# Zhang-Xiaoxue/Senquential-Convex-Programming-for-Trajectory-Planning

Measured on AMD Instinct MI355X. Metric: SCP-QP solves/sec/GPU (4 veh, Hp=20); traj ℓ∞ err vs CVXOPT, higher is better.
Workload: dtype f64; 1 GPU; c2: 4-vehicle circle/crossing, Hp=20, batch=1024 noise seeds per GPU, full SCP solve per problem; n_veh=4, hp=20, batch_per_gpu=1024, parallelism=1 independent shards (no collective)

## Files before the change

### senquential-convex-programming-for-trajectory-planning_amd/csrc/scpqp_kernel.h

```cpp

#pragma once

#include <hip/hip_runtime.h>

#include <math.h>
#include <stdint.h>
#include <stdio.h>
#include <stdlib.h>
#include <string.h>

#include <new>
#include <type_traits>
#include <utility>

#include "scpqp.h"

#define NT 256
#define TXD 16
#define TYD (NT / TXD)
#define NWAVE (NT / 64)
#define SCR_PER_WAVE 640

namespace {

// ... 675 lines not shown
            if (lane < 2 && act) L.p0[(v * Hb + k) * 2 + lane] = cur;
        }
        bar();
    }
    for (int e = tid; e < V * Hb; e += NT) {
        const int v = e / Hb, l = e % Hb;
        double acc = 0.0;
        for (int k = l; k < Hb; ++k) {
            const double qk = (k == Hb - 1) ? P.Qf[v] : P.Q[v];
            const ldouble* gg = L.g + (v * Hb + k - l) * 2;
            const double ex = L.ref[(v * Hb + k) * 2] - L.p0[(v * Hb + k) * 2];
            const double ey = L.ref[(v * Hb + k) * 2 + 1] - L.p0[(v * Hb + k) * 2 + 1];
            acc += qk * (gg[0] * ex + gg[1] * ey);
        }
        L.qs[e] = P.uLim * (-2.0 * acc);
    }
    for (int r = tid; r < L.m; r += NT) {
        int i, j, o, k;
        if (r < L.mp) {
            const int pi = r / Hb;
            k = r % Hb;
            int ii = 0, rem = pi;
            while (rem >= V - 1 - ii) { rem -= V - 1 - ii; ++ii; }
            i = ii;
            j = ii + 1 + rem;
            o = -1;
        } else {
            const int ro = r - L.mp;
            const int vo = ro / Hb;
            k = ro % Hb;
            i = vo / O;
            o = vo % O;
            j = -1;
        }
        L.rinfo[r] = i | ((j + 1) << 8) | ((o + 1) << 16) | (k << 24);
    }
    bar();
    return sflag;
}

template <bool HG, bool VG, int RM, int OCC, int SH>
__device__ __noinline__ int setup_problem_ni(const cKArgs* ap, const cParams* Pp, gdouble* ws, int b, int Hb) {
    ap = (const cKArgs*)readfirstlane_u64((unsigned long long)ap);
    Pp = (const cParams*)readfirstlane_u64((unsigned long long)Pp);
    ws = (gdouble*)readfirstlane_u64((unsigned long long)ws);
    b = __builtin_amdgcn_readfirstlane(b);
    Hb = __builtin_amdgcn_readfirstlane(Hb);
    const cKArgs& a = *ap;
    const cParams& P = *Pp;
    const Off f = plan_offsets(shapeV<SH>(P.nV), shapeO<SH>(P.nO), shapeHM<SH>(P.hpMax), HG, VG, lean_plan(HG, VG, OCC));
    const Lay<HG, VG, RM, OCC> L = make_lay<HG, VG, RM, OCC, SH>(lds_base(), ws, f, P.nV, P.nO, Hb);
    return setup_problem(a, P, L, b);
}

constexpr int kSplit = 3, kPerWave = 21, kPerPass = kPerWave * NWAVE;
template <class TermSum, class Fn>
__device__ __forceinline__ void split3_outputs(int nout, TermSum part, Fn fn, int w) {
    const int lane = threadIdx.x & 63;
    const int j = lane / kSplit, sidx = lane - j * kSplit;
    for (int base = 0; base < nout; base += kPerPass) {
        const int e = base + w * kPerWave + j;
        const bool valid = lane < kSplit * kPerWave && e < nout;
        double2v acc = valid ? part(e, sidx) : double2v{0.0, 0.0};
        const double x1 = __shfl_down(acc.x, 1), y1 = __shfl_down(acc.y, 1);
        const double x2 = __shfl_down(acc.x, 2), y2 = __shfl_down(acc.y, 2);
        if (valid && sidx == 0) fn(e, double2v{acc.x + x1 + x2, acc.y + y1 + y2});
    }
}
template <class TermSum, class Fn>
__device__ __forceinline__ void split3_outputs(int nout, TermSum part, Fn fn) {
    split3_outputs(nout, part, fn, (int)(threadIdx.x >> 6));
}

template <class LT, class PX, class PY>
__device__ __forceinline__ void toeplitz_apply(const LT& L, PX x, PY y) {
    split3_outputs(
        L.V * L.Hb,
        [&](int e, int sidx) {
            const int v = e / L.Hb, k = e - v * L.Hb;
            const ldouble* gv = L.g + v * L.Hb * 2;
            const int xb = v * L.Hb;
            double a0 = 0.0, a1 = 0.0;
            for (int l = sidx; l <= k; l += kSplit) {
                const double xl = x[xb + l];
                const double2v gl = ld2(gv + (k - l) * 2);
                a0 += gl.x * xl;
                a1 += gl.y * xl;
            }
            return double2v{a0, a1};
        },
        [&](int e, double2v r) { st2(y + 2 * e, r); });
}

template <class LT, class PY, class Fn>
__device__ __forceinline__ void toeplitz_t_apply(const LT& L, PY y, Fn out, int w) {
    split3_outputs(
        L.V * L.Hb,
        [&](int e, int sidx) {
            const int v = e / L.Hb, l = e - v * L.Hb;
            const ldouble* gv = L.g + v * L.Hb * 2;
            const int yb = v * L.Hb * 2;
            double acc = 0.0;
            for (int k = l + sidx; k < L.Hb; k += kSplit)
                acc += gv[(k - l) * 2] * y[yb + 2 * k] + gv[(k - l) * 2 + 1] * y[yb + 2 * k + 1];
            return double2v{acc, 0.0};
        },
        [&](int e, double2v r) { out(e, r.x); }, w);
}
template <class LT, class PY, class Fn>
__device__ __forceinline__ void toeplitz_t_apply(const LT& L, PY y, Fn out) {
    toeplitz_t_apply(L, y, out, (int)(threadIdx.x >> 6));
}

template <class LT, class F>
__device__ __forceinline__ void incident_sum(const LT& L, int v, int k, F coef, double& s0,
                                            double& s1) {
    s0 = 0.0;
    s1 = 0.0;
    for (int w = 0; w < L.V; ++w) {
        if (w == v) continue;
        const int i = v < w ? v : w, j = v < w ? w : v;
        const int r = pair_index(i, j, L.V) * L.Hb + k;
        const double c = (v == i ? -1.0 : 1.0) * coef(r);
        s0 += c * L.rowE[2 * r];
        s1 += c * L.rowE[2 * r + 1];
    }
    for (int o = 0; o < L.O; ++o) {
        const int r = L.mp + (v * L.O + o) * L.Hb + k;
        const double c = -coef(r);
        s0 += c * L.rowE[2 * r];
        s1 += c * L.rowE[2 * r + 1];
    }
}

template <class LT, class PX>
__device__ __forceinline__ double gx_row(const LT& L, PX xu, double xw, int r) {
    if (r < L.m) {
        int i, j, o, k;
        row_decode(L.rinfo[r], i, j, o, k);
        const double e0 = L.rowE[2 * r], e1 = L.rowE[2 * r + 1];
        double val = -(e0 * L.ya[(i * L.Hb + k) * 2] + e1 * L.ya[(i * L.Hb + k) * 2 + 1]);
        if (j >= 0) val += e0 * L.ya[(j * L.Hb + k) * 2] + e1 * L.ya[(j * L.Hb + k) * 2 + 1];
        return val + L.rowW[r] * xw;
    }
    if (r < L.m + L.N) return xu[r - L.m];
    if (r < L.m + 2 * L.N) return -xu[r - L.m - L.N];
    return -xw;
}

template <class LT, class PT>
__device__ __forceinline__ double gt_incident_part(const LT& L, PT t, int vt) {
    double wsum = 0.0;
    for (int e = vt; e < L.V * L.Hb; e += NT) {
        const int v = e / L.Hb, k = e % L.Hb;
        double s0, s1;
        incident_sum(L, v, k, [&](int r) { return t[r]; }, s0, s1);
        L.yb[2 * e] = s0;
        L.yb[2 * e + 1] = s1;
    }
    for (int r = vt; r < L.m; r += NT) wsum += t[r] * L.rowW[r];
    return wsum;
}
template <class LT, class PT, class Fin>
__device__ __forceinline__ void gt_toeplitz_part(const LT& L, PT t, Fin fin, int vw) {
    toeplitz_t_apply(L, L.yb, [&](int e, double tt) { fin(e, tt + t[L.m + e] - t[L.m + L.N + e]); }, vw);
}
template <int BUF, class LT, class PT, class Fin>
__device__ double gt_apply_fin(const LT& L, PT t, Fin fin) {
    const int tid = threadIdx.x;
    const double wsum = gt_incident_part(L, t, tid);
    double red[4] = {wsum, 0.0, 0.0, 0.0};
    block_reduce4<1, BUF>(red, 0, L.red);
    gt_toeplitz_part(L, t, fin, tid >> 6);
    return red[0] - t[L.mc - 1];
}

template <class LT, class PT, class Fin, class FinW>
struct GtSide {
    static constexpr int STAGES = 2;
    const LT& L;
    PT t;
    Fin fin;
    FinW finw;
    __device__ __forceinline__ void operator()(int stage, int h, int nh) const {
        const int lane = threadIdx.x & 63;
        ldouble* part = L.red + kSidePart;
        for (int vw = h; vw < NWAVE; vw += nh) {
            if (stage == 0) {
                const double ws = wave_sum(gt_incident_part(L, t, vw * 64 + lane));
                if (lane == 0) part[vw] = ws;
            } else {
                gt_toeplitz_part(L, t, fin, vw);
                if (vw == 0 && lane == 0) {
                    double r = part[0];
#pragma unroll
                    for (int ww = 1; ww < NWAVE; ++ww) r = r + part[ww];
                    finw(r - t[L.mc - 1]);
                }
            }
        }
    }
};
template <class LT, class PT, class Fin, class FinW>
__device__ __forceinline__ GtSide<LT, PT, Fin, FinW> gt_side(const LT& L, PT t, Fin fin, FinW finw) {
    return GtSide<LT, PT, Fin, FinW>{L, t, fin, finw};
}

template <int TS, class LT, class PD>
__device__ __forceinline__ void assemble_tiles(const cParams& P, const LT& L, PD d, double rho) {
    const int tid = threadIdx.x, V = L.V, Hb = L.Hb, nb = L.nb, N = L.N;
    const double u2 = P.uLim * P.uLim;
    const int TH = (Hb + TS - 1) / TS, TD = TH * (TH + 1) / 2, TO = TH * TH;
    const int PV = V * (V - 1) / 2;
    const int ntile = V * TD + PV * TO;
    const double2v zero2 = {0.0, 0.0};
    for (int r0 = 0; r0 < ntile; r0 += NT) {
        const int t = r0 + (((r0 / NT) & 1) ? NT - 1 - tid : tid);
        if (t >= ntile) continue;
        int a_, b_, lt, mt;
        tile_decode(t, V, PV, a_, b_, lt, mt);
        const int l0 = TS * lt, m0 = TS * mt, k0 = l0 > m0 ? l0 : m0;
        const ldouble* ga = L.g + a_ * Hb * 2;
        const ldouble* gb = L.g + b_ * Hb * 2;
        const auto* W = L.Wt + 4 * (a_ * (a_ + 1) / 2 + b_);
        double2v av[TS], bv[TS];
#pragma unroll
        for (int i = 0; i < TS; ++i) {
            const int ia = k0 - 1 - l0 - i, ib = k0 - 1 - m0 - i;
            av[i] = ia >= 0 ? ld2(ga + 2 * ia) : zero2;
            bv[i] = ib >= 0 ? ld2(gb + 2 * ib) : zero2;
        }
        double c[TS][TS];
#pragma unroll
        for (int i = 0; i < TS; ++i)
#pragma unroll
            for (int j = 0; j < TS; ++j) c[i][j] = 0.0;
        double2v an = ld2(ga + 2 * (k0 - l0)), bn = ld2(gb + 2 * (k0 - m0));
        double2v wn0 = ld2(W + 4 * k0 * nb), wn1 = ld2(W + 4 * k0 * nb + 2);
        constexpr bool PF2 = LT::HGLOBAL;
        double2v an2 = an, bn2 = bn, wm0 = wn0, wm1 = wn1;
        if constexpr (PF2) {
            const int k1 = k0 + 1 < Hb ? k0 + 1 : k0;
            an2 = ld2(ga + 2 * (k1 - l0));
            bn2 = ld2(gb + 2 * (k1 - m0));
            wm0 = ld2(W + 4 * k1 * nb);
            wm1 = ld2(W + 4 * k1 * nb + 2);
        }
        auto trip = [&](const double2v& anew, const double2v& bnew, const double2v& w0,
                        const double2v& w1) {
#pragma unroll
            for (int i = TS - 1; i > 0; --i) {
                av[i] = av[i - 1];
                bv[i] = bv[i - 1];
            }
            av[0] = anew;
            bv[0] = bnew;
            double px[TS], py[TS];
#pragma unroll
            for (int j = 0; j < TS; ++j) {
                px[j] = w0.x * bv[j].x + w0.y * bv[j].y;
                py[j] = w1.x * bv[j].x + w1.y * bv[j].y;
            }
#pragma unroll
            for (int i = 0; i < TS; ++i)
#pragma unroll
                for (int j = 0; j < TS; ++j) c[i][j] = fma(av[i].y, py[j], fma(av[i].x, px[j], c[i][j]));
        };
#pragma unroll 2
        for (int k = k0; k < Hb; ++k) {
            const double2v acur = an, bcur = bn, w0 = wn0, w1 = wn1;
            if constexpr (PF2) {
                an = an2;
                bn = bn2;
                wn0 = wm0;
                wn1 = wm1;
                const int kn = k + 2 < Hb ? k + 2 : Hb - 1;
                an2 = ld2(ga + 2 * (kn - l0));
                bn2 = ld2(gb + 2 * (kn - m0));
                wm0 = ld2(W + 4 * kn * nb);
                wm1 = ld2(W + 4 * kn * nb + 2);
            } else {
                const int kn = k + 1 < Hb ? k + 1 : k;
                an = ld2(ga + 2 * (kn - l0));
                bn = ld2(gb + 2 * (kn - m0));
                wn0 = ld2(W + 4 * kn * nb);
                wn1 = ld2(W + 4 * kn * nb + 2);
            }
            trip(acur, bcur, w0, w1);
        }
#pragma unroll
        for (int di = 0; di < TS; ++di)
#pragma unroll
            for (int dj = 0; dj < TS; ++dj) {
                const int l = l0 + di, lp = m0 + dj;
                if (l >= Hb || lp >= Hb || (a_ == b_ && lp > l)) continue;
                const int row = a_ * Hb + l, col = b_ * Hb + lp;
                double acc = c[di][dj];
                if (row == col) acc += 2.0 * u2 * P.R[a_] + d[L.m + row] + d[L.m + N + row] + rho;
                L.H[roff(row) + col] = acc;
            }
    }
}

template <class LT, class PD>
__device__ void assemble(const cParams& P, const LT& L, PD d, double rho) {
    const int tid = threadIdx.x, V = L.V, Hb = L.Hb, nb = L.nb;
    const double u2 = P.uLim * P.uLim;
    const int nW = Hb * nb;
    PROF_T0_FINE();
    for (int e = tid; e < nW + V * Hb; e += NT) {
        if (e < nW) {
            const int k = e / nb, ab = e % nb;
            int a_ = 0;
            while ((a_ + 1) * (a_ + 2) / 2 <= ab) ++a_;
            const int b_ = ab - a_ * (a_ + 1) / 2;
            double w00 = 0.0, w01 = 0.0, w11 = 0.0;
            if (a_ == b_) {
                const double qk = 2.0 * u2 * ((k == Hb - 1) ? P.Qf[a_] : P.Q[a_]);
                w00 = qk;
                w11 = qk;
                for (int wv = 0; wv < V; ++wv) {
                    if (wv == a_) continue;
                    const int i = a_ < wv ? a_ : wv, j = a_ < wv ? wv : a_;
                    const int r = pair_index(i, j, V) * Hb + k;
                    const double e0 = L.rowE[2 * r], e1 = L.rowE[2 * r + 1], dr = d[r];
                    w00 += dr * e0 * e0;
                    w01 += dr * e0 * e1;
                    w11 += dr * e1 * e1;
                }
                for (int o = 0; o < L.O; ++o) {
                    const int r = L.mp + (a_ * L.O + o) * Hb + k;
                    const double e0 = L.rowE[2 * r], e1 = L.rowE[2 * r + 1], dr = d[r];
                    w00 += dr * e0 * e0;
                    w01 += dr * e0 * e1;
                    w11 += dr * e1 * e1;
                }
            } else {
                const int r = pair_index(b_, a_, V) * Hb + k;
                const double e0 = L.rowE[2 * r], e1 = L.rowE[2 * r + 1], dr = -d[r];
                w00 = dr * e0 * e0;
                w01 = dr * e0 * e1;
                w11 = dr * e1 * e1;
            }
            auto* W = L.Wt + 4 * e;
            W[0] = w00; W[1] = w01; W[2] = w01; W[3] = w11;
        } else {
            const int q = e - nW, v = q / Hb, k = q % Hb;
            double s0, s1;
            incident_sum(L, v, k, [&](int r) { return d[r] * L.rowW[r]; }, s0, s1);
            L.yb[2 * q] = s0;
            L.yb[2 * q + 1] = s1;
        }
    }
    double ww = 0.0;
    for (int r = tid; r < L.m; r += NT) ww += d[r] * L.rowW[r] * L.rowW[r];
    double red[4] = {ww, 0.0, 0.0, 0.0};
    block_reduce4<1, 2>(red, 0, L.red);
    PROF_ACC_FINE0(25);
    const int T4 = (Hb + 3) >> 2, PV = V * (V - 1) / 2;
    if constexpr (LT::HGLOBAL) {
        if (V * (T4 * (T4 + 1) / 2) + PV * T4 * T4 >= 2 * NT) assemble_tiles<4>(P, L, d, rho);
        else assemble_tiles<2>(P, L, d, rho);
    } else {
        (void)T4;
        (void)PV;
        assemble_tiles<4>(P, L, d, rho);
#ifdef SCPQP_DIAG_X2_ASM
        assemble_tiles<4>(P, L, d, rho);
#endif
    }
    PROF_ACC_FINE0(26);
    const int N = L.N;
    toeplitz_t_apply(L, L.yb, [&](int e, double tt) { L.H[roff(N) + e] = tt; });
    if (tid == 0) L.H[roff(N) + N] = red[0] + d[L.mc - 1] + rho;
    bar();
    PROF_ACC_FINE0(27);
}

#define CB 8

__device__ __forceinline__ double recip(double x) {
    double r = __builtin_amdgcn_rcp(x);
    double e = fma(-x, r, 1.0);
    r = fma(r, e, r);
    e = fma(-x, r, 1.0);
    return fma(r, e, r);
}

__device__ __forceinline__ bool wave0() {
    return __builtin_amdgcn_readfirstlane(threadIdx.x) < 64;
}
__device__ __forceinline__ int wave_id() {
    return __builtin_amdgcn_readfirstlane(threadIdx.x) >> 6;
}
__device__ __forceinline__ bool is_lead(int lead) { return wave_id() == lead; }
__device__ __forceinline__ void lead_prio_up() { __builtin_amdgcn_s_setprio(2); }
__device__ __forceinline__ void lead_prio_down() { __builtin_amdgcn_s_setprio(0); }

template <int RS, bool OPQ, class HP>
__device__ __forceinline__ int panel_factor(HP H, ldouble* dinv, int n, int r0, int jb, int jp,
                                              const ldouble* dprev, ldouble* dout, lint* flag,
                                              int nprev, ldouble* ldbuf) {
    int lane = threadIdx.x & 63;
    if constexpr (OPQ) asm volatile("" : "+v"(lane));
    PROF_T0_FINE();
    double p[RS][CB];
    int ro[RS];
#pragma unroll
    for (int t = 0; t < RS; ++t) {
        const int i = r0 + lane + 64 * t;
        ro[t] = roff(i < n ? i : n - 1);
#pragma unroll
        for (int c = 0; c < CB; c += 2) {
            const double2v v = ld2(H + ro[t] + r0 + c);
            p[t][c] = v.x;
            p[t][c + 1] = v.y;
        }
    }
#ifdef SCPQP_PROF_FINE
    __builtin_amdgcn_s_waitcnt(0);
#endif
    PROF_ACC_FINE(18);
    for (int q = 0; jp >= 0 && q < nprev; ++q) {
        double li[RS][CB];
#pragma unroll
        for (int t = 0; t < RS; ++t)
#pragma unroll
            for (int c = 0; c < CB; c += 2) {
                const double2v v = ld2(H + ro[t] + jp + q * CB + c);
                li[t][c] = v.x;
                li[t][c + 1] = v.y;
            }
        if (q == nprev - 1) {
#pragma unroll
            for (int c = 0; c < CB; c += 2) {
                double lk0[CB], lk1[CB];
#pragma unroll
                for (int c2 = 0; c2 < CB; c2 += 2) {
                    const double2v v0 = ld2(ldbuf + c * CB + c2), v1 = ld2(ldbuf + (c + 1) * CB + c2);
                    lk0[c2] = v0.x; lk0[c2 + 1] = v0.y;
                    lk1[c2] = v1.x; lk1[c2 + 1] = v1.y;
                }
#pragma unroll
                for (int t = 0; t < RS; ++t) {
                    double s0 = li[t][0] * lk0[0], s1 = li[t][0] * lk1[0];
#pragma unroll
                    for (int c2 = 1; c2 < CB; ++c2) {
                        s0 = fma(li[t][c2], lk0[c2], s0);
                        s1 = fma(li[t][c2], lk1[c2], s1);
                    }
                    p[t][c] -= s0;
                    p[t][c + 1] -= s1;
                }
            }
        } else {
            double ld[CB];
#pragma unroll
            for (int c = 0; c < CB; ++c) ld[c] = li[0][c] * dprev[q * CB + c];
#pragma unroll
            for (int c = 0; c < CB; ++c) {
                double lk[CB];
#pragma unroll
                for (int c2 = 0; c2 < CB; ++c2) lk[c2] = readlane_d(ld[c2], c);
#pragma unroll
                for (int t = 0; t < RS; ++t) {
                    double sacc = 0.0;
#pragma unroll
                    for (int c2 = 0; c2 < CB; c2 += 2) sacc += li[t][c2] * lk[c2] + li[t][c2 + 1] * lk[c2 + 1];
                    p[t][c] -= sacc;
                }
            }
        }
    }
    if (jb < CB) {
#pragma unroll
        for (int t = 0; t < RS; ++t) {
            const int i = r0 + lane + 64 * t;
#pragma unroll
            for (int c = 0; c < CB; ++c)
                p[t][c] = (i < n && c < jb) ? p[t][c] : ((t == 0 && lane == c) ? 1.0 : 0.0);
        }
    }
    PROF_ACC_FINE(19);
    if (jb == 1) {
        const double D = readlane_d(p[0][0], 0);
        const int bad1 = !(D > 0.0) || !isfinite(D);
        if (lane == 0) {
            dinv[r0] = recip(D);
            dout[0] = D;
            flag[0] = bad1;
        }
        return bad1;
    }
    double inv[CB], dg[CB];
    int bad = 0;
    double u0[CB];
#pragma unroll
    for (int c = 0; c < CB; c += 2) {
        double U0[CB], V[CB], W[CB];
#pragma unroll
        for (int c2 = c; c2 < CB; ++c2) U0[c2] = readlane_d(p[0][c], c2);
#pragma unroll
        for (int c2 = c + 1; c2 < CB; ++c2) V[c2] = readlane_d(p[0][c + 1], c2);
        const double d0 = U0[c], b = U0[c + 1], e = V[c + 1];
        const double det = fma(d0, e, -(b * b));
        const double i0 = recip(d0), rdet = recip(det);
        const double i1 = d0 * rdet;
        dg[c] = d0;
        dg[c + 1] = det * i0;
        bad |= !(d0 > 0.0) || !isfinite(d0) || !(det > 0.0) || !isfinite(det);
        inv[c] = i0;
        inv[c + 1] = i1;
#pragma unroll
        for (int c2 = c + 2; c2 < CB; ++c2) W[c2] = fma(-(U0[c2] * i0), b, V[c2]);
        u0[c] = p[0][c];
#pragma unroll
        for (int t = 0; t < RS; ++t) {
            const double l0 = p[t][c] * i0;
            const double pc1 = fma(-l0, b, p[t][c + 1]);
            if (t == 0) u0[c + 1] = pc1;
            const double l1 = pc1 * i1;
#pragma unroll
            for (int c2 = c + 2; c2 < CB; ++c2) p[t][c2] = fma(-l1, W[c2], fma(-l0, U0[c2], p[t][c2]));
            p[t][c] = l0;
            p[t][c + 1] = l1;
        }
    }
    if (lane < CB && lane < jb) {
        double iv = inv[0], dv = dg[0];
#pragma unroll
        for (int c = 1; c < CB; ++c) {
            iv = lane == c ? inv[c] : iv;
            dv = lane == c ? dg[c] : dv;
        }
        dinv[r0 + lane] = iv;
        dout[lane] = dv;
    }
    PROF_ACC_FINE(20);
#pragma unroll
    for (int t = 0; t < RS; ++t) {
        const int i = r0 + lane + 64 * t;
        if (i < n) {
#pragma unroll
            for (int c = 0; c < CB; c += 2)
                if (c < jb && c <= lane + 64 * t) st2(H + ro[t] + r0 + c, double2v{p[t][c], p[t][c + 1]});
        }
    }
    if (lane >= CB && lane < 2 * CB) {
#pragma unroll
        for (int c = 0; c < CB; c += 2) st2(ldbuf + (lane - CB) * CB + c, double2v{u0[c], u0[c + 1]});
    }
    if (lane == 0) flag[0] = bad;
    PROF_ACC_FINE(21);
    return bad;
}

template <class HP, bool NEUTRAL = false>
__device__ __forceinline__ void trailing_update(HP H, int n, int j0, int r1, const ldouble* dcur,
                                                int t0, int nth) {
    double dc[CB];
#pragma unroll
    for (int c = 0; c < CB; ++c) dc[c] = dcur[c];
    const int T = (n - r1 + 1) >> 1;
    const int ntile = T * (T + 1) / 2;
    for (int t = t0; t < ntile; t += 2 * nth) {
        const int tb = t + nth < ntile ? t + nth : t;
        int ia[2], ka[2];
        tri_decode(t, ia[0], ka[0]);
        tri_decode(tb, ia[1], ka[1]);
        double sm[2][4];
#pragma unroll
        for (int u2 = 0; u2 < 2; ++u2) {
            const int o0 = roff(r1 + 2 * ia[u2]), o1 = roff(r1 + 2 * ia[u2] + 1);
            const int q0 = roff(r1 + 2 * ka[u2]), q1 = roff(r1 + 2 * ka[u2] + 1);
            double s00 = 0.0, s01 = 0.0, s10 = 0.0, s11 = 0.0;
#pragma unroll
            for (int c = 0; c < CB; c += 2) {
                const double2v x0 = ld2(H + o0 + j0 + c), x1 = ld2(H + o1 + j0 + c);
                const double2v y0 = ld2(H + q0 + j0 + c), y1 = ld2(H + q1 + j0 + c);
                const double e0 = x0.x * dc[c], e1 = x0.y * dc[c + 1];
                const double f0 = x1.x * dc[c], f1 = x1.y * dc[c + 1];
                s00 = fma(e1, y0.y, fma(e0, y0.x, s00));
                s01 = fma(e1, y1.y, fma(e0, y1.x, s01));
                s10 = fma(f1, y0.y, fma(f0, y0.x, s10));
                s11 = fma(f1, y1.y, fma(f0, y1.x, s11));
            }
            sm[u2][0] = s00; sm[u2][1] = s01; sm[u2][2] = s10; sm[u2][3] = s11;
        }
#pragma unroll
        for (int u2 = 0; u2 < 2; ++u2) {
            if (u2 == 1 && tb == t) break;
            const int i0 = r1 + 2 * ia[u2], k0 = r1 + 2 * ka[u2];
            const int o0 = roff(i0), o1 = roff(i0 + 1);
            const double f = NEUTRAL ? 0.0 : 1.0;
            H[o0 + k0] -= f * sm[u2][0];
            H[o0 + k0 + 1] -= f * sm[u2][1];
            H[o1 + k0] -= f * sm[u2][2];
            H[o1 + k0 + 1] -= f * sm[u2][3];
        }
    }
}

typedef double double4v __attribute__((ext_vector_type(4)));

template <int U, int KS, class HP>
__device__ __forceinline__ void trailing_update_mfma(HP H, int n, int j0, int r1, const ldouble* dcur,
                                                     int wave, int nwave, int part = 0, int np = 1) {
    const int lane = threadIdx.x & 63, lr = lane & 15, lk = lane >> 4;
    double dk[KS];
#pragma unroll
    for (int kk = 0; kk < KS; ++kk) dk[kk] = dcur[4 * kk + lk];
    const int T = (n - r1 + 15) >> 4;
    const int ntile = T * (T + 1) / 2;
    int tb = 0, te = ntile;
    if (part != 0) {
        int js = 1, cum = T;
        for (int k = 1; k < np; ++k) {
            while (js < T && np * cum < k * ntile) {
                cum += T - js;
                ++js;
            }
            if (k == part - 1) tb = cum;
            if (k == part) te = cum;
        }
    }
    for (int t = tb + wave; t < te; t += U * nwave) {
        double a[U][KS], b[U][KS];
        double4v acc[U];
        int oc[U][4];
        bool ok[U][4];
#pragma unroll
        for (int u = 0; u < U; ++u) {
            const int tu = t + u * nwave;
            const bool live = tu < te;
            int I = 0, J = 0;
            tri_decode(ntile - 1 - (live ? tu : t), J, I);
            I = T - 1 - I;
            J = T - 1 - J;
            const int i0 = r1 + 16 * I, k0 = r1 + 16 * J;
            const int ia = min(i0 + lr, n - 1), kb = min(k0 + lr, n - 1);
            const int oa = roff(ia) + j0, ob = roff(kb) + j0;
#pragma unroll
            for (int kk = 0; kk < KS; ++kk) {
                a[u][kk] = -H[oa + 4 * kk + lk] * dk[kk];
                b[u][kk] = H[ob + 4 * kk + lk];
            }
            const int kc = k0 + lr;
#pragma unroll
            for (int r = 0; r < 4; ++r) {
                const int ci = i0 + lk + 4 * r;
                ok[u][r] = live && ci < n && kc <= ci;
                oc[u][r] = roff(ok[u][r] ? ci : 0) + (ok[u][r] ? kc : 0);
                acc[u][r] = ok[u][r] ? (double)H[oc[u][r]] : 0.0;
            }
        }
#pragma unroll
        for (int u = 0; u < U; ++u) {
#pragma unroll
            for (int kk = 0; kk < KS; ++kk)
                acc[u] = __builtin_amdgcn_mfma_f64_16x16x4f64(a[u][kk], b[u][kk], acc[u], 0, 0, 0);
        }
#pragma unroll
        for (int u = 0; u < U; ++u)
#pragma unroll
            for (int r = 0; r < 4; ++r)
                if (ok[u][r]) H[oc[u][r]] = acc[u][r];
    }
}

constexpr int kGroup = 4;
static_assert(kPivSlot + 2 * kGroup * CB == red_size(true) && kPivSlot + 2 * CB == red_size(false),
              "the pivot buffer of red_size");
static_assert(kSidePart > kIdlSlot && kSidePart + NWAVE <= kPivSlot,
              "the side job's partials lie between the polish slot and the pivots");

struct NoSide {
    static constexpr int STAGES = 0;
    __device__ __forceinline__ void operator()(int, int, int) const {}
};
// ... 745 lines not shown
    double mrd = 0.0, quad2 = 0.0, lin = 0.0;
    toeplitz_t_apply(L, L.yb, [&](int e, double tt) {
        const int v = e / Hb;
        const double ze = L.z[e];
        const double pu = 2.0 * u2 * P.R[v] * ze;
        const double rde = tt + pu + L.qs[e] + L.lam[L.m + e] - L.lam[L.m + N + e];
        L.rd[e] = rde;
        mrd = fmax(mrd, fabs(rde));
        quad2 += pu * ze;
        lin += L.qs[e] * ze;
    });
    const double rdw = P.slackW + red[2] - L.lam[L.mc - 1];
    if (tid == 0) L.rd[N] = rdw;
    double red2[4] = {mrd, quad2, lin, 0.0};
    block_reduce4<3, 1>(red2, 1, L.red);
    out[0] = red[0];
    out[1] = fmax(red2[0], fabs(rdw));
    out[2] = red[1];
    out[3] = 0.5 * (red[3] + red2[1]) + red2[2] + P.slackW * zw;
}

struct Ctx {
    const cParams* P;
    gdouble* ws;
    int Hb, lead;
};
struct D4 {
    double a, b, c, d;
};

constexpr double kPolishTol = 1e-9;
__device__ __forceinline__ int polish_stop(const D4& d, int ref, double early) {
    if (ref < 1) return 0;
    if (d.a <= kPolishTol * fmax(1.0, d.b)) return 1;
    if (d.c > early || d.d > early) return 2;
    return 0;
}

__device__ __forceinline__ Ctx uniform_ctx(const Ctx& c) {
    Ctx u;
    u.P = (const cParams*)readfirstlane_u64((unsigned long long)c.P);
    u.ws = (gdouble*)readfirstlane_u64((unsigned long long)c.ws);
    u.Hb = __builtin_amdgcn_readfirstlane(c.Hb);
    u.lead = __builtin_amdgcn_readfirstlane(c.lead);
    return u;
}

template <bool HG, bool VG, int RM, int OCC, int SH>
__device__ __forceinline__ Lay<HG, VG, RM, OCC> lay_of(const Ctx& c) {
    const Off f = plan_offsets(shapeV<SH>(c.P->nV), shapeO<SH>(c.P->nO), shapeHM<SH>(c.P->hpMax), HG, VG, lean_plan(HG, VG, OCC));
    Lay<HG, VG, RM, OCC> L = make_lay<HG, VG, RM, OCC, SH>(lds_base(), c.ws, f, c.P->nV, c.P->nO, c.Hb);
    L.lead = c.lead;
    return L;
}
#define PHASE template <bool HG, bool VG, int RM, int OCC, int SH> __device__ __noinline__
#define LAYDEF                  \
    const Ctx cu_ = uniform_ctx(c); \
    const cParams& P = *cu_.P;  \
    const Lay<HG, VG, RM, OCC> L = lay_of<HG, VG, RM, OCC, SH>(cu_); \
    (void)P
#define PH(f) f<HG, VG, RM, OCC, SH>
#define PH_FWD(f) f<HG, VG, RM, OCC, SH, kRhsOverlap && !HG, kFwdSweep<HG, SH>>
#define ROWSDEF RowsOf<SH, Lay<HG, VG, RM, OCC>> A{L}

PHASE void ph_solve(Ctx c, int dst) {
    LAYDEF;
    chol_solve<SH>(L, L.rhs, dst ? L.dz : L.z);
}
PHASE void ph_solve_back(Ctx c, int dst) {
    LAYDEF;
    chol_solve_back<SH>(L, dst ? L.dz : L.z);
}
template <int SH>
__device__ __forceinline__ const double* uniform_margin(const double* mg) {
    if constexpr (shape_c(SH).V != 0) return nullptr;
    else return (const double*)readfirstlane_u64((unsigned long long)mg);
}
PHASE int ph_margin_bad(Ctx c, const double* mg_) {
    LAYDEF;
    const double* mg = uniform_margin<SH>(mg_);
    lint* orslot = (lint*)(L.red + kOrSlot);
    if (threadIdx.x == 0) *orslot = 0;
    bar();
    bool bad = false;
    if (mg)
        for (int i = threadIdx.x; i < L.O * L.Hb; i += NT) bad |= !(mg[i] >= 0.0) || mg[i] == INFINITY;
    if (bad) *orslot = 1;
    bar();
    const int any = __builtin_amdgcn_readfirstlane(*orslot);
    bar();
    return any;
}
PHASE void ph_linearise(Ctx c, const double* mg) {
    LAYDEF;
    linearise_rows(P, L, uniform_margin<SH>(mg));
}
PHASE EvalRes ph_evaluate(Ctx c, double* cveh, double* cobs, const double* mg) {
    LAYDEF;
    return evaluate_u(P, L, L.ub, cveh, cobs, uniform_margin<SH>(mg));
}
PHASE D4 ph_residuals(Ctx c) {
    LAYDEF;
    ROWSDEF;
    A.template load<RV_S | RV_LAM>();
    double r[4];
    residuals(P, L, A, r);
    return D4{r[0], r[1], r[2], r[3]};
}
template <class LT>
__device__ __forceinline__ void rhs_from_tv_body(const cParams& P, const LT& L, double rho) {
    const double ow = gt_apply_fin<1>(L, L.tv, [&](int e, double g) { L.rhs[e] = g - L.qs[e] + rho * L.dz[e]; });
    if (threadIdx.x == 0) L.rhs[L.N] = ow - P.slackW + rho * L.dz[L.N];
    bar();
}
template <class LT>
__device__ __forceinline__ auto rhs_from_tv_side(const cParams& P, const LT& L, double rho) {
    return gt_side(
        L, L.tv, [&L, rho](int e, double g) { L.rhs[e] = g - L.qs[e] + rho * L.dz[e]; },
        [&L, &P, rho](double ow) { L.rhs[L.N] = ow - P.slackW + rho * L.dz[L.N]; });
}
#ifdef SCPQP_DIAG_RHS_FRONT
constexpr bool kRhsOverlap = false;
#else
constexpr bool kRhsOverlap = true;
#endif
#define PHASE_OVL                                                                     \
    template <bool HG, bool VG, int RM, int OCC, int SH, bool OVL = kRhsOverlap && !HG, \
              bool FWD = false>                                                        \
    __device__ __noinline__
PHASE void ph_fwd_sweep_step(Ctx c, int s, int dst) {
    LAYDEF;
    FwdSide<shape_n<SH>(), Lay<HG, VG, RM, OCC>>{L, dst ? L.dz : L.z}(__builtin_amdgcn_readfirstlane(s));
}
template <bool HG, bool VG, int RM, int OCC, int SH>
struct FwdCall {
    static constexpr bool ON = true;
    static_assert(fwd_fits<HG, SH>(), "FWD only where the sweep fits");
    Ctx c;
    int dst;
    __device__ __forceinline__ void operator()(int s) const {
        if (s > FwdSide<shape_n<SH>(), Lay<HG, VG, RM, OCC>>::S1) PH(ph_fwd_sweep_step)(c, s, dst);
    }
};
#define FWD_CALL(dst) FwdCall<HG, VG, RM, OCC, SH>{cu_, dst}
template <bool HG, int SH>
constexpr bool kFwdSweep = kFwdOverlap && kRhsOverlap && fwd_fits<HG, SH>();
PHASE void ph_rhs_from_tv(Ctx c, double rho) {
    LAYDEF;
    rhs_from_tv_body(P, L, rho);
}
PHASE void ph_init_a(Ctx c) {
    LAYDEF;
    const int tid = threadIdx.x;
    for (int r = tid; r < L.mc; r += NT) {
        L.dd[r] = 1.0;
        L.tv[r] = hval(L, r);
    }
    for (int e = tid; e < L.n; e += NT) L.dz[e] = 0.0;
    bar();
}
PHASE void ph_init_b(Ctx c) {
    LAYDEF;
    const int tid = threadIdx.x, N = L.N, mc = L.mc;
    toeplitz_apply(L, L.z, L.ya);
    bar();
    double vmax = 0.0;
    for (int r = tid; r < L.m; r += NT) {
        const double gu = gx_row(L, L.z, 0.0, r);
        L.s[r] = gu;
        vmax = fmax(vmax, (gu - L.rowH[r]) / -L.rowW[r]);
    }
    double red[4] = {vmax, 0.0, 0.0, 0.0};
    block_reduce4<1>(red, 1, L.red);
    const double om = red[0] + 1.0;
    double smin = 1e300, smax = -1e300;
    for (int r = tid; r < mc; r += NT) {
        const double gx = r < L.m ? L.s[r] + L.rowW[r] * om : gx_row(L, L.z, om, r);
        const double sv = hval(L, r) - gx;
        L.s[r] = sv;
        smin = fmin(smin, sv);
        smax = fmax(smax, sv);
    }
    double red2[4] = {-smin, smax, 0.0, 0.0};
    block_reduce4<2, 1>(red2, 3, L.red);
    const double ts = fmax(1.5 * red2[0], 0.0);
    const double fl = 0.1 * fmax(1.0, red2[1] + ts);
    const double lam0 = 0.3 * P.slackW / mc;
    for (int r = tid; r < mc; r += NT) {
        L.s[r] = fmax(L.s[r] + ts, fl);
        L.lam[r] = r == mc - 1 ? P.slackW : lam0;
    }
    if (tid == 0) L.z[N] = om;
    bar();
}
template <bool TV = true, class LT, class RW>
__device__ __forceinline__ void newton_rhs_body(const LT& L, RW& A, int corr, double smu) {
    if constexpr (TV) {
        each_row(A, L.mc, [&](int k, int r) {
            const double rc = A.s(k, r) * A.lam(k, r) + (corr ? A.sa(k, r) * A.la(k, r) - smu : 0.0);
            L.tv[r] = A.dd(k, r) * A.rp(k, r) - rc * recip(A.s(k, r));
        });
        bar();
    }
    const double ow = gt_apply_fin<0>(L, L.tv, [&](int e, double g) { L.rhs[e] = -L.rd[e] - g; });
    if (threadIdx.x == 0) L.rhs[L.N] = -L.rd[L.N] - ow;
    bar();
}
template <class LT>
__device__ __forceinline__ auto newton_rhs_side(const LT& L) {
    return gt_side(
        L, L.tv, [&L](int e, double g) { L.rhs[e] = -L.rd[e] - g; },
        [&L](double ow) { L.rhs[L.N] = -L.rd[L.N] - ow; });
}
template <class LT, class RW>
__device__ __forceinline__ double2v newton_back_body(const LT& L, RW& A, int corr, double smu) {
    toeplitz_apply(L, L.dz, L.ya);
    bar();
    const double xw = L.dz[L.N];
    double ap = 1.0, ad = 1.0;
    each_row(A, L.mc, [&](int k, int r) {
        const double rc = A.s(k, r) * A.lam(k, r) + (corr ? A.sa(k, r) * A.la(k, r) - smu : 0.0);
        const double dsr = -A.rp(k, r) - gx_row(L, L.dz, xw, r);
        const double dlr = -(rc + A.lam(k, r) * dsr) * recip(A.s(k, r));
        A.ds(k, r) = dsr;
        A.dl(k, r) = dlr;
        if (dsr < 0.0) ap = fmin(ap, -A.s(k, r) * recip(dsr));
        if (dlr < 0.0) ad = fmin(ad, -A.lam(k, r) * recip(dlr));
    });
    return double2v{ap, ad};
}
template <class LT, class RW>
__device__ __forceinline__ double affine_body(const LT& L, RW& A, double mu, double2v part) {
    double redm[4] = {-fmin(part.x, part.y), 0.0, 0.0, 0.0};
    block_reduce4<1>(redm, 1, L.red);
    const double aaff = -redm[0];
    double mua = 0.0;
    each_row(A, L.mc, [&](int k, int r) {
        mua += (A.s(k, r) + aaff * A.ds(k, r)) * (A.lam(k, r) + aaff * A.dl(k, r));
    });
    double red[4] = {mua, 0.0, 0.0, 0.0};
    block_reduce4<1, 1>(red, 0, L.red);
    const double sr = red[0] / L.mc / mu;
    return sr * sr * sr * mu;
}
template <class LT, class RW>
__device__ __forceinline__ void update_body(const LT& L, RW& A, double eta, double2v part) {
    double ap = part.x, ad = part.y;
    double red[4] = {-ap, -ad, 0.0, 0.0};
    block_reduce4<2>(red, 3, L.red);
    ap = fmin(1.0, eta * -red[0]);
    ad = fmin(1.0, eta * -red[1]);
    for (int e = threadIdx.x; e < L.n; e += NT) L.z[e] += ap * L.dz[e];
    each_row(A, L.mc, [&](int k, int r) {
        A.s(k, r) += ap * A.ds(k, r);
        A.lam(k, r) += ad * A.dl(k, r);
    });
    A.template store<RV_S | RV_LAM>();
    bar();
}
__device__ __forceinline__ double step_factor(double mu) { return fmax(0.99, 1.0 - mu); }
template <class LT, class RW>
__device__ __forceinline__ void polish_tv_pass(const LT& L, RW& A) {
    const double idl = L.red[kIdlSlot];
    each_row(A, L.mc, [&](int k, int r) { L.tv[r] = A.sa(k, r) * (hval(L, r) * idl - A.la(k, r)); });
}
PHASE_OVL int ph_scale_assemble_rhs_factor(Ctx c) {
    LAYDEF;
    PROF_T0_FINE();
    assemble(P, L, L.dd, 0.0);
    PROF_ACC_FINE0(29);
    if constexpr (OVL && FWD) {
        return cholesky(L, newton_rhs_side(L), FWD_CALL(1)) ? 1 : 0;
    } else if constexpr (OVL) {
        if (side_fits<2>(L)) return cholesky(L, newton_rhs_side(L)) ? 1 : 0;
    }
    RowsMem<Lay<HG, VG, RM, OCC>> A{L};
    newton_rhs_body<false>(L, A, 0, 0.0);
    PROF_ACC_FINE0(28);
    return cholesky(L) ? 1 : 0;
}
PHASE_OVL int ph_assemble_factor(Ctx c, double rho) {
    LAYDEF;
    if constexpr (OVL) {
        {
            ROWSDEF;
            A.template load<RV_SA | RV_LA>();
            polish_tv_pass(L, A);
        }
        assemble(P, L, L.dd, rho);
        if constexpr (FWD) {
            return cholesky(L, rhs_from_tv_side(P, L, P.polRho), FWD_CALL(1)) ? 1 : 0;
        }
        if (side_fits<2>(L)) return cholesky(L, rhs_from_tv_side(P, L, P.polRho)) ? 1 : 0;
        if (!cholesky(L)) return 0;
        rhs_from_tv_body(P, L, P.polRho);
        return 1;
    } else {
        assemble(P, L, L.dd, rho);
        return cholesky(L) ? 1 : 0;
    }
}
PHASE_OVL void ph_init_assemble_factor(Ctx c) {
    LAYDEF;
    assemble(P, L, L.dd, 0.0);
    const int N = L.N, o = roff(N);
    for (int e = threadIdx.x; e <= N; e += NT) L.H[o + e] = e == N ? 1.0 : 0.0;
    bar();
    if constexpr (OVL && FWD) {
        cholesky(L, rhs_from_tv_side(P, L, 0.0), FWD_CALL(0));
    } else if constexpr (OVL) {
        if (side_fits<2>(L)) {
            cholesky(L, rhs_from_tv_side(P, L, 0.0));
        } else {
            cholesky(L);
            rhs_from_tv_body(P, L, 0.0);
        }
    } else {
        cholesky(L);
    }
}
PHASE double ph_back_affine_rhs(Ctx c, double mu) {
    LAYDEF;
    ROWSDEF;
    A.template load<RV_S | RV_LAM | RV_RP | RV_DD>();
    const double2v part = newton_back_body(L, A, 0, 0.0);
    const double smu = affine_body(L, A, mu, part);
    A.template store<RV_SA | RV_LA>();
    newton_rhs_body(L, A, 1, smu);
    return smu;
}
PHASE D4 ph_back_update_residuals(Ctx c, double smu, double eta) {
    LAYDEF;
    ROWSDEF;
    A.template load<RV_S | RV_LAM | RV_RP | RV_SA | RV_LA>();
    const double2v part = newton_back_body(L, A, 1, smu);
    update_body(L, A, eta, part);
    double r[4];
    residuals(P, L, A, r);
    return D4{r[0], r[1], r[2], r[3]};
}
PHASE void ph_polish_prep(Ctx c) {
    LAYDEF;
    const double idl = 1.0 / P.polDelta;
    if (threadIdx.x == 0) L.red[kIdlSlot] = idl;
    for (int r = threadIdx.x; r < L.mc; r += NT) {
        const bool act = L.lam[r] > L.s[r];
        L.dd[r] = act ? idl : 0.0;
        L.la[r] = act ? L.lam[r] : 0.0;
        L.sa[r] = act ? 1.0 : 0.0;
    }
    for (int e = threadIdx.x; e < L.n; e += NT) L.dz[e] = L.rd[e] = L.z[e];
    bar();
}
PHASE void ph_polish_warm(Ctx c) {
    LAYDEF;
    const double idl = 1.0 / P.polDelta;
    if (threadIdx.x == 0) L.red[kIdlSlot] = idl;
    for (int r = threadIdx.x; r < L.mc; r += NT) L.dd[r] = L.sa[r] != 0.0 ? idl : 0.0;
    for (int e = threadIdx.x; e < L.n; e += NT) L.dz[e] = L.rd[e] = L.z[e];
    bar();
}
PHASE D4 ph_scales(Ctx c) {
    LAYDEF;
    const int tid = threadIdx.x;
    double hmax = 1.0;
    for (int r = tid; r < L.m; r += NT) hmax = fmax(hmax, fabs(L.rowH[r]));
    double qmax = fmax(1.0, P.slackW);
    for (int e = tid; e < L.N; e += NT) qmax = fmax(qmax, fabs(L.qs[e]));
    double red[4] = {hmax, qmax, 0.0, 0.0};
    block_reduce4<2>(red, 3, L.red);
    return D4{red[0], red[1], 0.0, 0.0};
}
template <class LT, class RW>
__device__ __forceinline__ void polish_rhs_body(const cParams& P, const LT& L, RW& A) {
    polish_tv_pass(L, A);
    bar();
    rhs_from_tv_body(P, L, P.polRho);
}
PHASE void ph_polish_rhs(Ctx c) {
    LAYDEF;
    ROWSDEF;
    A.template load<RV_SA | RV_LA>();
    polish_rhs_body(P, L, A);
}
template <class LT, class RW>
__device__ __forceinline__ D4 polish_dual_body(const cParams& P, const LT& L, RW& A) {
    const double idl = L.red[kIdlSlot];
    toeplitz_apply(L, L.dz, L.ya);
    bar();
    const double xw = L.dz[L.N];
    double viol = -1e300, yneg = -1e300;
    each_row(A, L.mc, [&](int k, int r) {
        const double hr = hval(L, r);
        const double rpr = gx_row(L, L.dz, xw, r) - hr;
        A.rp(k, r) = rpr;
        const double sar = A.sa(k, r);
        double y = A.la(k, r);
        if (sar != 0.0) {
            y = y + rpr * idl;
            A.la(k, r) = y;
            yneg = fmax(yneg, -y);
        } else {
            viol = fmax(viol, rpr);
        }
        L.tv[r] = sar * (hr * idl - y);
    });
    A.template store<RV_RP | RV_LA>();
    double dmax = 0.0, xmax = 0.0;
    for (int e = threadIdx.x; e < L.n; e += NT) {
        const double x = L.dz[e];
        dmax = fmax(dmax, fabs(x - L.rd[e]));
        xmax = fmax(xmax, fabs(x));
        L.rd[e] = x;
    }
    double red[4] = {dmax, xmax, viol, yneg};
    block_reduce4<4>(red, 15, L.red);
    return D4{red[0], red[1], red[2], red[3]};
}
PHASE D4 ph_polish_dual_next(Ctx c, int ref, int cap, double early) {
    LAYDEF;
    ROWSDEF;
    A.template load<RV_SA | RV_LA>();
    const D4 d = polish_dual_body(P, L, A);
    if (polish_stop(d, ref, early) == 0 && ref + 1 < cap) rhs_from_tv_body(P, L, P.polRho);
    return d;
}
PHASE int ph_polish_accept(Ctx c, double hmax, int converged) {
    LAYDEF;
    const int tid = threadIdx.x;
    double viol = -1e300, ymin = 1e300, ymax = 0.0, nonfin = 0.0;
    for (int r = tid; r < L.mc; r += NT) {
        viol = fmax(viol, L.rp[r]);
        if (L.sa[r] != 0.0) {
            ymin = fmin(ymin, L.la[r]);
            ymax = fmax(ymax, fabs(L.la[r]));
        }
    }
    for (int e = tid; e < L.n; e += NT)
        if (!isfinite(L.dz[e])) nonfin = 1.0;
    double red[4] = {viol, -ymin, ymax, nonfin};
    block_reduce4<4, 1>(red, 15, L.red);
    const double vtol = 1e-9 * hmax, ytol = -1e-9 * fmax(1.0, red[2]);
    const bool ok = converged && red[0] <= vtol && -red[1] >= ytol && red[3] == 0.0;
    if (ok) {
        for (int e = tid; e < L.n; e += NT) L.z[e] = L.dz[e];
        bar();
        return 1;
    }
    if (red[3] != 0.0) return 0;
    const double idl = L.red[kIdlSlot];
    double changed = 0.0;
    for (int r = tid; r < L.mc; r += NT) {
        const bool act = L.sa[r] != 0.0;
        const bool add = !act && L.rp[r] > vtol;
        const bool drop = act && L.la[r] < ytol;
        if (add || drop) {
            changed += 1.0;
            L.sa[r] = add ? 1.0 : 0.0;
            L.la[r] = 0.0;
            L.dd[r] = add ? idl : 0.0;
        }
    }
    double red2[4] = {changed, 0.0, 0.0, 0.0};
    block_reduce4<1>(red2, 0, L.red);
    return red2[0] != 0.0 ? 1 + (int)red2[0] : 0;
}
PHASE void ph_take_u(Ctx c) {
    LAYDEF;
    for (int i = threadIdx.x; i < L.N; i += NT) L.ub[i] = P.uLim * L.z[i];
    bar();
}

PHASE void ph_trace_rows(Ctx c, double* dst) {
    LAYDEF;
    for (int i = threadIdx.x; i < L.N; i += NT) dst[kTraceHdr + i] = L.ub[i];
    const int N2 = kTraceHdr + 2 * P.nV * P.hpMax;
    for (int r = threadIdx.x; r < L.m; r += NT) {
        dst[N2 + 4 * r] = L.rowE[2 * r];
        dst[N2 + 4 * r + 1] = L.rowE[2 * r + 1];
        dst[N2 + 4 * r + 2] = L.rowW[r];
        dst[N2 + 4 * r + 3] = L.rowH[r];
    }
}
PHASE void ph_trace_sol(Ctx c, double* dst, D4 ev, double delta, int ipm, int qfl, double merit0,
                        int rounds, int refines) {
    LAYDEF;
    for (int i = threadIdx.x; i < L.N; i += NT) dst[kTraceHdr + P.nV * P.hpMax + i] = L.ub[i];
    if (threadIdx.x == 0) {
        dst[8] = merit0;
        dst[9] = rounds + 4096.0 * refines;
        dst[0] = delta;
        dst[1] = ev.a;
        dst[2] = ev.b;
        dst[3] = ev.c;
        dst[4] = L.z[L.N];
        dst[5] = ipm;
        dst[6] = qfl;
        dst[7] = ev.d;
    }
}

constexpr int kPolishRounds = 6;
constexpr int kWarmRounds = 8;
constexpr int kWarmRefine = 12;
constexpr double kWarmEarly = 1e-6;
constexpr bool kWarmStall = true;

struct QpStats {
    int ipm, rounds, refine, warm_ok;
};

template <bool HG, bool VG, int RM, int OCC, int SH>
__device__ __forceinline__ bool polish_rounds(Ctx c, double hmax, double rho, int max_rounds,
                                              int cap, double early, QpStats& st, bool stall = false) {
    bool ok = false, refactor = true, extended = false;
    int prev_chg = 1 << 30;
    PROF_T0();
    for (int round = 0; round < max_rounds && !ok; ++round) {
        ++st.rounds;
        if (refactor) {
            const bool fact = PH_FWD(ph_assemble_factor)(c, rho) != 0;
            PROF_ACC(7);
            if (!fact) break;
        }
        int conv = 0;
        if (!(kRhsOverlap && !HG) || !refactor) PH(ph_polish_rhs)(c);
        for (int ref = 0; ref < cap; ++ref) {
            bool back = false;
            if constexpr (kFwdSweep<HG, SH>) {
                back = refactor && ref == 0;
                if (back) PH(ph_solve_back)(c, 1);
            }
            if (!back) PH(ph_solve)(c, 1);
            const D4 d = PH(ph_polish_dual_next)(c, ref, cap, early);
            ++st.refine;
            const int stop = polish_stop(d, ref, early);
            conv = stop == 1;
            if (stop) break;
        }
        const int acc = PH(ph_polish_accept)(c, hmax, conv);
        PROF_ACC(8);
        ok = acc == 1;
        if (acc == 0 && (conv || extended)) break;
        if (acc >= 2) {
            if (stall && round >= 1 && acc - 1 >= prev_chg) break;
            prev_chg = acc - 1;
        }
        extended |= acc == 0;
        refactor = acc >= 2;
    }
    return ok;
}

struct QpKnobs {
    int maxIpm, nRefine, mc;
    double ipmTol, polRho;
};
template <bool HG, bool VG, int RM, int OCC, int SH>
__device__ __forceinline__ bool qp_solve_body(Ctx c, const QpKnobs& K, int& qflags, bool warm,
                                              QpStats& st) {
    const int mc = K.mc;
    const D4 sc = PH(ph_scales)(c);
    const double hmax = sc.a, qmax = sc.b;
    if (warm) {
        PH(ph_polish_warm)(c);
        if (polish_rounds<HG, VG, RM, OCC, SH>(c, hmax, K.polRho, kWarmRounds, kWarmRefine, kWarmEarly,
                                               st, kWarmStall)) {
            ++st.warm_ok;
            return true;
        }
    }
    PROF_T0();
    PH(ph_init_a)(c);
    PH_FWD(ph_init_assemble_factor)(c);
    if constexpr (!(kRhsOverlap && !HG)) PH(ph_rhs_from_tv)(c, 0.0);
    if constexpr (kFwdSweep<HG, SH>) PH(ph_solve_back)(c, 0);
    else PH(ph_solve)(c, 0);
    PH(ph_init_b)(c);
    PROF_ACC(16);
    int it = 0;
    bool conv = false, ok = false, maxit = false;
    double tol = K.ipmTol;
    D4 res = PH(ph_residuals)(c);
    PROF_ACC(1);
    for (int pass = 0;; ++pass) {
        for (; it < K.maxIpm; ++it) {
            PROF_ACC(0);
            if (res.a <= tol * hmax && res.b <= tol * qmax && res.c <= tol * fmax(1.0, fabs(res.d))) {
                conv = true;
                break;
            }
            const double mu = res.c / mc;
            if (!PH_FWD(ph_scale_assemble_rhs_factor)(c)) break;
            PROF_ACC(3);
            if constexpr (kFwdSweep<HG, SH>) PH(ph_solve_back)(c, 1);
            else PH(ph_solve)(c, 1);
            PROF_ACC(9);
            const double smu = PH(ph_back_affine_rhs)(c, mu);
            PROF_ACC(5);
            PH(ph_solve)(c, 1);
            PROF_ACC(9);
            res = PH(ph_back_update_residuals)(c, smu, step_factor(mu));
            PROF_ACC(6);
        }
        if (pass == 0 && !conv && it >= K.maxIpm) maxit = true;
        PH(ph_polish_prep)(c);
        ok = polish_rounds<HG, VG, RM, OCC, SH>(c, hmax, K.polRho, kPolishRounds, K.nRefine, INFINITY, st);
        if (ok || !conv || pass == 1) break;
        tol *= 0.01;
        conv = false;
// ... 298 lines not shown
```

Before: 148,500 SCP solves/s.

## Fuse incident-sum into diagonal W assembly and split omega row across waves

```diff
diff --git a/senquential-convex-programming-for-trajectory-planning_amd/csrc/scpqp_kernel.h b/senquential-convex-programming-for-trajectory-planning_amd/csrc/scpqp_kernel.h
--- a/senquential-convex-programming-for-trajectory-planning_amd/csrc/scpqp_kernel.h
+++ b/senquential-convex-programming-for-trajectory-planning_amd/csrc/scpqp_kernel.h
@@ -1001,13 +1001,22 @@
     }
 }
 
+#ifdef SCPQP_DIAG_ASM_FRONT
+constexpr bool kAsmOverlap = false;
+#else
+constexpr bool kAsmOverlap = true;
+#endif
+constexpr bool kAsmFuseYb = kAsmOverlap;
+constexpr bool kAsmOmegaBeside = kAsmOverlap;
+constexpr int kAsmOmegaWaves = 2;
+
 template <class LT, class PD>
 __device__ void assemble(const cParams& P, const LT& L, PD d, double rho) {
     const int tid = threadIdx.x, V = L.V, Hb = L.Hb, nb = L.nb;
     const double u2 = P.uLim * P.uLim;
     const int nW = Hb * nb;
     PROF_T0_FINE();
-    for (int e = tid; e < nW + V * Hb; e += NT) {
+    for (int e = tid; e < (kAsmFuseYb ? nW : nW + V * Hb); e += NT) {
         if (e < nW) {
             const int k = e / nb, ab = e % nb;
             int a_ = 0;
@@ -1018,6 +1027,8 @@
                 const double qk = 2.0 * u2 * ((k == Hb - 1) ? P.Qf[a_] : P.Q[a_]);
                 w00 = qk;
                 w11 = qk;
+                constexpr bool yb_here = kAsmFuseYb;
+                double s0 = 0.0, s1 = 0.0;
                 for (int wv = 0; wv < V; ++wv) {
                     if (wv == a_) continue;
                     const int i = a_ < wv ? a_ : wv, j = a_ < wv ? wv : a_;
@@ -1026,6 +1037,11 @@
                     w00 += dr * e0 * e0;
                     w01 += dr * e0 * e1;
                     w11 += dr * e1 * e1;
+                    if constexpr (yb_here) {
+                        const double c = (a_ == i ? -1.0 : 1.0) * (dr * L.rowW[r]);
+                        s0 += c * e0;
+                        s1 += c * e1;
+                    }
                 }
                 for (int o = 0; o < L.O; ++o) {
                     const int r = L.mp + (a_ * L.O + o) * Hb + k;
@@ -1033,7 +1049,19 @@
                     w00 += dr * e0 * e0;
                     w01 += dr * e0 * e1;
                     w11 += dr * e1 * e1;
+                    if constexpr (yb_here) {
+                        const double c = -(dr * L.rowW[r]);
+                        s0 += c * e0;
+                        s1 += c * e1;
+                    }
                 }
+                if constexpr (yb_here) {
+                    const int q = a_ * Hb + k;
+                    L.yb[2 * q] = s0;
+                    L.yb[2 * q + 1] = s1;
+                }
+                (void)s0;
+                (void)s1;
             } else {
                 const int r = pair_index(b_, a_, V) * Hb + k;
                 const double e0 = L.rowE[2 * r], e1 = L.rowE[2 * r + 1], dr = -d[r];
@@ -1068,12 +1096,30 @@
         assemble_tiles<4>(P, L, d, rho);
 #endif
     }
-    PROF_ACC_FINE0(26);
     const int N = L.N;
-    toeplitz_t_apply(L, L.yb, [&](int e, double tt) { L.H[roff(N) + e] = tt; });
-    if (tid == 0) L.H[roff(N) + N] = red[0] + d[L.mc - 1] + rho;
+    {
+        bool beside = false;
+        if constexpr (kAsmOmegaBeside && !LT::HGLOBAL)
+            beside = V * (T4 * (T4 + 1) / 2) + PV * T4 * T4 <= NT;
+        auto orow = [&](int e, double tt) { L.H[roff(N) + e] = tt; };
+        PROF_ACC_FINE0(26);
+        if (beside) {
+            const int w = __builtin_amdgcn_readfirstlane(tid >> 6) - (NWAVE - kAsmOmegaWaves);
+            for (int vw = w; vw >= 0 && vw < NWAVE; vw += kAsmOmegaWaves) toeplitz_t_apply(L, L.yb, orow, vw);
+        } else {
+            toeplitz_t_apply(L, L.yb, orow);
+        }
+        if (tid == 0) L.H[roff(N) + N] = red[0] + d[L.mc - 1] + rho;
+    }
     bar();
     PROF_ACC_FINE0(27);
+}
+template <class LT>
+__device__ __forceinline__ void assemble_cold(const cParams& P, const LT& L) {
+    assemble(P, L, L.dd, 0.0);
+    const int N = L.N, o = roff(N);
+    for (int e = threadIdx.x; e <= N; e += NT) L.H[o + e] = e == N ? 1.0 : 0.0;
+    bar();
 }
 
 #define CB 8
@@ -2425,10 +2471,7 @@
 }
 PHASE_OVL void ph_init_assemble_factor(Ctx c) {
     LAYDEF;
-    assemble(P, L, L.dd, 0.0);
-    const int N = L.N, o = roff(N);
-    for (int e = threadIdx.x; e <= N; e += NT) L.H[o + e] = e == N ? 1.0 : 0.0;
-    bar();
+    assemble_cold(P, L);
     if constexpr (OVL && FWD) {
         cholesky(L, rhs_from_tv_side(P, L, 0.0), FWD_CALL(0));
     } else if constexpr (OVL) {
```

After: 151,400 SCP solves/s, median of 6. +1.9%, better.
